# MDFahimAnjum/AliasFree-Diffusion-Models-PyTorch

Measured on AMD Instinct MI355X. Metric: train_step_images_per_sec, higher is better.
Workload: dtype f32; 1 GPU; CIFAR-10 32x32x3 synthetic, UNet variant=3 (Config D), batch 256/GPU, T=1000, AdamW lr 3e-4, random-init weights (seed 42); global_batch=256, parallelism=dp1, hip_graph=True, launch_mode=lanes

## Files before the change

aliasfree-diffusion-models-pytorch_amd/csrc/attn.hip:

```cpp
#include "attn_forms.h"

namespace afd {

constexpr int kTile = 64;
constexpr int kChunk = 8;

using f2 = __attribute__((ext_vector_type(2))) float;
constexpr float kLog2e = 1.4426950408889634f, kLn2 = 0.6931471805599453f;

template <int D> struct RowVec {
  static __device__ __forceinline__ void load(const float* __restrict__ p, f2 (&v)[D / 2]) {
    if constexpr (D % 4 == 0) {
#pragma unroll
      for (int j = 0; j < D / 4; ++j) {
        const float4 t = reinterpret_cast<const float4*>(p)[j];
        v[2 * j] = (f2){t.x, t.y}; v[2 * j + 1] = (f2){t.z, t.w};
      }
    } else {
      const float2 t = *reinterpret_cast<const float2*>(p);
      v[0] = (f2){t.x, t.y};
    }
  }
};
template <int P> __device__ __forceinline__ float dot2(const f2 (&a)[P], const f2 (&b)[P]) {
// ... 145 lines not shown
      const float g = live ? d_o[obase + (long)j * L + qi] : 0.f;
      q[r][j >> 1][j & 1] = live ? qp[(long)j * L + qi] * (scale * kLog2e) : 0.f;
      go[r][j >> 1][j & 1] = g;
      delta[r] += g * (live ? o[obase + (long)j * L + qi] : 0.f);
    }
#pragma unroll
    for (int i = 0; i < P; ++i) dq[r][i] = (f2){0.f, 0.f};
    ls[r] = live ? lse[((long)b * heads + h) * L + qi] * kLog2e : 0.f;
    if (live) delta_out[((long)b * heads + h) * L + qi] = delta[r];
  }
  for (int k0 = 0; k0 < L; k0 += kTile) {
    __syncthreads();
    stage_rows<D, NT>(kp, Ks, k0, L, 1.f);
    stage_rows<D, NT>(vp, Vs, k0, L, 1.f);
    __syncthreads();
    const int nk = min(kTile, L - k0);
#pragma unroll 2
    for (int u = 0; u < nk; ++u) {
      f2 kv[P], vv[P];
      RowVec<D>::load(Ks + u * D, kv);
      RowVec<D>::load(Vs + u * D, vv);
#pragma unroll
      for (int r = 0; r < R; ++r) {
        const float sc = dot2<P>(q[r], kv), dp = dot2<P>(go[r], vv);
        const float ds = __builtin_amdgcn_exp2f(sc - ls[r]) * (dp - delta[r]);
        axpy2<P>(dq[r], ds, kv);
      }
    }
  }
#pragma unroll
  for (int r = 0; r < R; ++r) {
    const int qi = q0 + r * NT;
    if (qi < L) {
      float* dqp = dqkv + ((long)b * 3 * C + h * D) * L + qi;
#pragma unroll
      for (int j = 0; j < D; ++j) dqp[(long)j * L] = dq[r][j >> 1][j & 1] * scale;
    }
  }
}

template <int D, int R, int NT>
__global__ __launch_bounds__(NT) void attn_bwd_dkv_k(const float* __restrict__ qkv, const float* __restrict__ d_o,
                                                      const float* __restrict__ lse, const float* __restrict__ delta,
                                                      float* __restrict__ dqkv, int heads, int L, float scale) {
  constexpr int P = D / 2;
  __shared__ __attribute__((aligned(16))) float Qs[kTile * D];
  __shared__ __attribute__((aligned(16))) float Gs[kTile * D];
  __shared__ float Ls[kTile];
  __shared__ float Ds[kTile];
  const int b = blockIdx.z, h = blockIdx.y;
  const int C = heads * D;
  const int kq0 = blockIdx.x * NT * R + threadIdx.x;
  const float* qp = qkv + ((long)b * 3 * C + h * D) * L;
  const float* kp = qp + (long)C * L;
  const float* vp = kp + (long)C * L;
  const float* gp = d_o + ((long)b * C + h * D) * L;
  const float* lp = lse + ((long)b * heads + h) * L;
  const float* dlp = delta + ((long)b * heads + h) * L;
  f2 k[R][P], v[R][P], dk[R][P], dv[R][P];
#pragma unroll
  for (int r = 0; r < R; ++r) {
    const int ki = kq0 + r * NT;
#pragma unroll
    for (int j = 0; j < D; ++j) {
      k[r][j >> 1][j & 1] = ki < L ? kp[(long)j * L + ki] : 0.f;
      v[r][j >> 1][j & 1] = ki < L ? vp[(long)j * L + ki] : 0.f;
    }
#pragma unroll
    for (int i = 0; i < P; ++i) { dk[r][i] = (f2){0.f, 0.f}; dv[r][i] = (f2){0.f, 0.f}; }
  }
  for (int t0 = 0; t0 < L; t0 += kTile) {
    __syncthreads();
    stage_rows<D, NT>(qp, Qs, t0, L, scale * kLog2e);
    stage_rows<D, NT>(gp, Gs, t0, L, 1.f);
    for (int i = threadIdx.x; i < kTile; i += NT) {
      const bool in = t0 + i < L;
      Ls[i] = in ? lp[t0 + i] * kLog2e : INFINITY;
      Ds[i] = in ? dlp[t0 + i] : 0.f;
    }
    __syncthreads();
    const int nq = min(kTile, L - t0);
#pragma unroll 2
    for (int u = 0; u < nq; ++u) {
      f2 qv[P], gv[P];
      RowVec<D>::load(Qs + u * D, qv);
      RowVec<D>::load(Gs + u * D, gv);
      const float lsu = Ls[u], dlu = Ds[u];
#pragma unroll
      for (int r = 0; r < R; ++r) {
        const float sc = dot2<P>(qv, k[r]), dp = dot2<P>(gv, v[r]);
        const float p = __builtin_amdgcn_exp2f(sc - lsu);
        const float ds = p * (dp - dlu);
        axpy2<P>(dv[r], p, gv);
        axpy2<P>(dk[r], ds, qv);
      }
    }
  }
#pragma unroll
  for (int r = 0; r < R; ++r) {
    const int ki = kq0 + r * NT;
    if (ki < L) {
      float* dkp = dqkv + ((long)b * 3 * C + C + h * D) * L + ki;
      float* dvp = dkp + (long)C * L;
#pragma unroll
      for (int j = 0; j < D; ++j) { dkp[(long)j * L] = dk[r][j >> 1][j & 1] * kLn2; dvp[(long)j * L] = dv[r][j >> 1][j & 1]; }
    }
  }
}

}
using namespace afd;

template <int R> static inline void attn_geometry(int B, int heads, int L, dim3& grid, dim3& block) {
  const int rows = (L + R - 1) / R;
  block = dim3(rows <= 64 ? 64 : (rows <= 128 ? 128 : 256));
  grid = dim3((L + block.x * R - 1) / (block.x * R), heads, B);
}
template <int D, int R> static void launch_fwd(const float* qkv, float* o, float* lse, int B, int heads, int L, float sc, hipStream_t s) {
  dim3 grid, block; attn_geometry<R>(B, heads, L, grid, block);
  if (block.x == 64) hipLaunchKernelGGL((attn_fwd_k<D, R, 64>), grid, block, 0, s, qkv, o, lse, heads, L, sc);
  else if (block.x == 128) hipLaunchKernelGGL((attn_fwd_k<D, R, 128>), grid, block, 0, s, qkv, o, lse, heads, L, sc);
  else hipLaunchKernelGGL((attn_fwd_k<D, R, 256>), grid, block, 0, s, qkv, o, lse, heads, L, sc);
}
template <int D, int R> static void launch_dq(const float* qkv, const float* o, const float* d_o, const float* lse, float* dqkv,
                                              float* delta, int B, int heads, int L, float sc, hipStream_t s) {
  dim3 grid, block; attn_geometry<R>(B, heads, L, grid, block);
  if (block.x == 64) hipLaunchKernelGGL((attn_bwd_dq_k<D, R, 64>), grid, block, 0, s, qkv, o, d_o, lse, dqkv, delta, heads, L, sc);
  else if (block.x == 128) hipLaunchKernelGGL((attn_bwd_dq_k<D, R, 128>), grid, block, 0, s, qkv, o, d_o, lse, dqkv, delta, heads, L, sc);
  else hipLaunchKernelGGL((attn_bwd_dq_k<D, R, 256>), grid, block, 0, s, qkv, o, d_o, lse, dqkv, delta, heads, L, sc);
}
template <int D, int R> static void launch_dkv(const float* qkv, const float* d_o, const float* lse, const float* delta, float* dqkv,
                                               int B, int heads, int L, float sc, hipStream_t s) {
  dim3 grid, block; attn_geometry<R>(B, heads, L, grid, block);
  if (block.x == 64) hipLaunchKernelGGL((attn_bwd_dkv_k<D, R, 64>), grid, block, 0, s, qkv, d_o, lse, delta, dqkv, heads, L, sc);
  else if (block.x == 128) hipLaunchKernelGGL((attn_bwd_dkv_k<D, R, 128>), grid, block, 0, s, qkv, d_o, lse, delta, dqkv, heads, L, sc);
  else hipLaunchKernelGGL((attn_bwd_dkv_k<D, R, 256>), grid, block, 0, s, qkv, d_o, lse, delta, dqkv, heads, L, sc);
}

static int g_attn_mfma_bwd_all = 1;
static int g_attn_rows = 0;

static int g_attn_small = 1;
static inline bool attn_small_use(int B, int heads, int d, int L) {
  return g_attn_small && g_attn_rows == 0 && attn_small_ok(d, L) && (long)B * heads <= (1L << 30);
}

extern "C" {

int afd_debug_attn_rows(int r) {
  if (r == 20 || r == 21) { g_attn_pv = r - 20; return AFD_OK; }
  if (r == 40 || r == 41) { g_attn_pv16 = r - 40; return AFD_OK; }
  if (r == 30 || r == 31) { g_attn_small = r - 30; return AFD_OK; }
  if (r == 10 || r == 11) { g_attn_mfma_bwd_all = r - 10; return AFD_OK; }
  AFD_REQUIRE(r == 0 || r == 1 || r == 2 || r == 4, "afd_debug_attn_rows: r must be 0, 1, 2, 4 (rows per lane of the VALU kernels), 10, 11, 20, 21, 30, 31, 40 or 41");
  g_attn_rows = r;
  return AFD_OK;
}

int afd_attn_fwd(const float* qkv, float* o, float* lse, int B, int heads, int d, int L, afd_stream_t st) {
  AFD_REQUIRE(qkv && o && lse && B > 0 && heads > 0 && L > 0, "afd_attn_fwd: bad argument");
  AFD_REQUIRE(d == 2 || d == 4 || d == 8 || d == 16 || d == 32 || d == 64, "afd_attn_fwd: head dim %d not in {2,4,8,16,32,64}", d);
  AFD_REQUIRE(B <= 65535 && heads <= 65535, "afd_attn_fwd: grid too large");
  hipStream_t s = as_stream(st);
  const float sc = 1.0f / sqrtf((float)d);
  if (g_attn_rows == 0 && attn_mfma8_ok(d, L)) { attn_mfma8_fwd(qkv, o, lse, B, heads, d, L, sc, s); return check_launch("afd_attn_fwd"); }
  if (attn_small_use(B, heads, d, L) && aligned16(qkv)) {
    attn_small_fwd_launch(qkv, o, lse, B, heads, d, L, sc, s);
    return check_launch("afd_attn_fwd");
  }
  switch (d) {
    case 2:  launch_fwd<2, 4>(qkv, o, lse, B, heads, L, sc, s); break;
    case 4:  launch_fwd<4, 4>(qkv, o, lse, B, heads, L, sc, s); break;
    case 8:
      if (g_attn_rows == 1 || (g_attn_rows == 0 && L < 1024)) launch_fwd<8, 1>(qkv, o, lse, B, heads, L, sc, s);
      else if (g_attn_rows == 4) launch_fwd<8, 4>(qkv, o, lse, B, heads, L, sc, s);
      else launch_fwd<8, 2>(qkv, o, lse, B, heads, L, sc, s);
      break;
    case 16: if (L <= 64) launch_fwd<16, 1>(qkv, o, lse, B, heads, L, sc, s); else launch_fwd<16, 2>(qkv, o, lse, B, heads, L, sc, s); break;
    case 32: if (L <= 64) launch_fwd<32, 1>(qkv, o, lse, B, heads, L, sc, s); else launch_fwd<32, 2>(qkv, o, lse, B, heads, L, sc, s); break;
    default: launch_fwd<64, 1>(qkv, o, lse, B, heads, L, sc, s); break;
  }
  return check_launch("afd_attn_fwd");
}

int afd_attn_bwd(const float* qkv, const float* o, const float* d_o, const float* lse, float* dqkv, float* delta_ws,
                 int B, int heads, int d, int L, afd_stream_t st) {
  AFD_REQUIRE(qkv && o && d_o && lse && dqkv && delta_ws && B > 0 && heads > 0 && L > 0, "afd_attn_bwd: bad argument");
  AFD_REQUIRE(d == 2 || d == 4 || d == 8 || d == 16 || d == 32 || d == 64, "afd_attn_bwd: head dim %d not in {2,4,8,16,32,64}", d);
  AFD_REQUIRE(B <= 65535 && heads <= 65535, "afd_attn_bwd: grid too large");
  hipStream_t s = as_stream(st);
  const float sc = 1.0f / sqrtf((float)d);
  if (g_attn_rows == 0 && attn_mfma8_ok(d, L) && (L < 1024 || g_attn_mfma_bwd_all)) {
    if (attn_fused_bwd(qkv, o, d_o, lse, dqkv, delta_ws, B, heads, d, L, sc, s)) return check_launch("afd_attn_bwd");
    attn_mfma8_bwd_dq(qkv, o, d_o, lse, dqkv, delta_ws, B, heads, d, L, sc, s);
    if (d == 8) attn_mfma8_bwd_dkv(qkv, d_o, lse, delta_ws, dqkv, B, heads, L, sc, s);
    else launch_dkv<16, 2>(qkv, d_o, lse, delta_ws, dqkv, B, heads, L, sc, s);
    return check_launch("afd_attn_bwd");
  }
  if (attn_small_use(B, heads, d, L) && aligned16(qkv) && aligned16(d_o)) {
    attn_small_bwd_launch(qkv, d_o, dqkv, B, heads, d, L, sc, s);
    return check_launch("afd_attn_bwd");
  }
  switch (d) {
    case 2:  launch_dq<2, 4>(qkv, o, d_o, lse, dqkv, delta_ws, B, heads, L, sc, s); break;
    case 4:  launch_dq<4, 4>(qkv, o, d_o, lse, dqkv, delta_ws, B, heads, L, sc, s); break;
    case 8:
      if (g_attn_rows == 1 || (g_attn_rows == 0 && L < 1024)) launch_dq<8, 1>(qkv, o, d_o, lse, dqkv, delta_ws, B, heads, L, sc, s);
      else if (g_attn_rows == 4) launch_dq<8, 4>(qkv, o, d_o, lse, dqkv, delta_ws, B, heads, L, sc, s);
      else launch_dq<8, 2>(qkv, o, d_o, lse, dqkv, delta_ws, B, heads, L, sc, s);
      break;
    case 16: if (L <= 64) launch_dq<16, 1>(qkv, o, d_o, lse, dqkv, delta_ws, B, heads, L, sc, s); else launch_dq<16, 2>(qkv, o, d_o, lse, dqkv, delta_ws, B, heads, L, sc, s); break;
    case 32: if (L <= 64) launch_dq<32, 1>(qkv, o, d_o, lse, dqkv, delta_ws, B, heads, L, sc, s); else launch_dq<32, 2>(qkv, o, d_o, lse, dqkv, delta_ws, B, heads, L, sc, s); break;
    default: launch_dq<64, 1>(qkv, o, d_o, lse, dqkv, delta_ws, B, heads, L, sc, s); break;
  }
  switch (d) {
    case 2:  launch_dkv<2, 4>(qkv, d_o, lse, delta_ws, dqkv, B, heads, L, sc, s); break;
    case 4:  launch_dkv<4, 4>(qkv, d_o, lse, delta_ws, dqkv, B, heads, L, sc, s); break;
    case 8:
      if (g_attn_rows == 1 || (g_attn_rows == 0 && L < 1024)) launch_dkv<8, 1>(qkv, d_o, lse, delta_ws, dqkv, B, heads, L, sc, s);
      else if (g_attn_rows == 4) launch_dkv<8, 4>(qkv, d_o, lse, delta_ws, dqkv, B, heads, L, sc, s);
      else launch_dkv<8, 2>(qkv, d_o, lse, delta_ws, dqkv, B, heads, L, sc, s);
      break;
    case 16: if (L <= 64) launch_dkv<16, 1>(qkv, d_o, lse, delta_ws, dqkv, B, heads, L, sc, s); else launch_dkv<16, 2>(qkv, d_o, lse, delta_ws, dqkv, B, heads, L, sc, s); break;
    case 32: launch_dkv<32, 1>(qkv, d_o, lse, delta_ws, dqkv, B, heads, L, sc, s); break;
    default: launch_dkv<64, 1>(qkv, d_o, lse, delta_ws, dqkv, B, heads, L, sc, s); break;
  }
  return check_launch("afd_attn_bwd");
}

}
```

aliasfree-diffusion-models-pytorch_amd/csrc/attn_forms.h:

```cpp
#pragma once
#include "common.h"

namespace afd {

extern int g_attn_pv;
extern int g_attn_pv16;
bool attn_mfma8_ok(int d, int L);
bool attn_fused_bwd(const float* qkv, const float* o, const float* d_o, const float* lse, float* dqkv, float* delta, int B, int heads,
                    int d, int L, float sc, hipStream_t s);
void attn_mfma8_fwd(const float* qkv, float* o, float* lse, int B, int heads, int d, int L, float sc, hipStream_t s);
void attn_mfma8_bwd_dq(const float* qkv, const float* o, const float* d_o, const float* lse, float* dqkv, float* delta,
                       int B, int heads, int d, int L, float sc, hipStream_t s);
void attn_mfma8_bwd_dkv(const float* qkv, const float* d_o, const float* lse, const float* delta, float* dqkv, int B, int heads, int L,
                        float sc, hipStream_t s);

bool attn_small_ok(int d, int L);
void attn_small_fwd_launch(const float* qkv, float* o, float* lse, int B, int heads, int d, int L, float sc, hipStream_t s);
void attn_small_bwd_launch(const float* qkv, const float* d_o, float* dqkv, int B, int heads, int d, int L, float sc, hipStream_t s);

}
```

aliasfree-diffusion-models-pytorch_amd/csrc/attn_mfma.hip:

```cpp
#include "attn_forms.h"
#include "h2_common.h"

namespace afd {

using f32x16 = __attribute__((ext_vector_type(16))) float;
constexpr int kTK = 64;
constexpr float kLog2e = 1.4426950408889634f, kLn2 = 0.6931471805599453f;

__device__ __forceinline__ float xhalf(float v) { return __shfl_xor(v, 32, kWave); }
__device__ __forceinline__ int acc_row(int r, int half) { return (r & 3) + 8 * (r >> 2) + 4 * half; }

using f2 = __attribute__((ext_vector_type(2))) float;
template <int D>
__device__ __forceinline__ void load_row(const float* __restrict__ p, f2 (&v)[D / 2]) {
#pragma unroll
  for (int q = 0; q < D / 4; ++q) {
    const float4 a = reinterpret_cast<const float4*>(p)[q];
    v[2 * q] = (f2){a.x, a.y}; v[2 * q + 1] = (f2){a.z, a.w};
  }
}
template <int D>
__device__ __forceinline__ void axpy(f2 (&acc)[D / 2], float s, const f2 (&v)[D / 2]) {
  const f2 ss = {s, s};
#pragma unroll
  for (int i = 0; i < D / 2; ++i) acc[i] = __builtin_elementwise_fma(ss, v[i], acc[i]);
}

using bf8 = __attribute__((ext_vector_type(8))) __bf16;
using bf2 = __attribute__((ext_vector_type(2))) __bf16;
__device__ __forceinline__ void split3(float x, __bf16& a, __bf16& b, __bf16& c) {
  a = (__bf16)x; const float r = x - (float)a;
  b = (__bf16)r; const float r2 = r - (float)b;
  c = (__bf16)r2;
}
template <int D>
__device__ __forceinline__ void row_frags(const float (&x)[D], int half, bf8 (&f)[3]) {
  bf8 p1, p2, p3;
#pragma unroll
  for (int j = 0; j < 8; ++j) {
    __bf16 a, b, c;
    split3(D == 8 ? x[j] : (half ? x[(8 + j) % D] : x[j]), a, b, c);
    p1[j] = a; p2[j] = b; p3[j] = c;
  }
  if (D == 8) { f[0] = p1; f[1] = half ? p1 : p2; f[2] = half ? p3 : p2; }
  else { f[0] = p1; f[1] = p2; f[2] = p3; }
}
template <int D>
__device__ __forceinline__ void stage_pieces(uint32_t* __restrict__ P, int rr, int jp, float v0, float v1) {
  __bf16 a0, b0, c0, a1, b1, c1;
  split3(v0, a0, b0, c0); split3(v1, a1, b1, c1);
  const int rec = D == 8 ? rr : (jp >> 2) * kTK + rr, w = jp & 3, ps = (D / 8) * kTK;
  P[(0 * ps + rec) * 4 + w] = __builtin_bit_cast(uint32_t, (bf2){a0, a1});
  P[(1 * ps + rec) * 4 + w] = __builtin_bit_cast(uint32_t, (bf2){b0, b1});
  P[(2 * ps + rec) * 4 + w] = __builtin_bit_cast(uint32_t, (bf2){c0, c1});
}
template <int D>
__device__ __forceinline__ void load_frags(const uint32_t* __restrict__ P, int row, int half, bf8 (&a)[3]) {
  const bf8* p = reinterpret_cast<const bf8*>(P);
  if (D == 8) { a[0] = p[(half ? 1 : 0) * kTK + row]; a[1] = p[(half ? 2 : 0) * kTK + row]; a[2] = p[(half ? 0 : 1) * kTK + row]; }
  else {
#pragma unroll
    for (int m = 0; m < 3; ++m) a[m] = p[(m * 2 + half) * kTK + row];
  }
}
template <int D>
__device__ __forceinline__ f32x16 dotx3(const bf8 (&a)[3], const bf8 (&b)[3]) {
  f32x16 c;
#pragma unroll
  for (int r = 0; r < 16; ++r) c[r] = 0.f;
  if (D == 8) {
#pragma unroll
    for (int m = 0; m < 3; ++m) c = __builtin_amdgcn_mfma_f32_32x32x16_bf16(a[m], b[m], c, 0, 0, 0);
  } else {
    constexpr int TA[6] = {0, 1, 0, 2, 1, 0}, TB[6] = {0, 0, 1, 0, 1, 2};
#pragma unroll
    for (int m = 0; m < 6; ++m) c = __builtin_amdgcn_mfma_f32_32x32x16_bf16(a[TA[m]], b[TB[m]], c, 0, 0, 0);
  }
  return c;
}

template <int D>
__device__ __forceinline__ f32x16 dotx3c(const bf8 (&a)[3], const bf8 (&b)[3], f32x16 c) {
  if (D == 8) {
#pragma unroll
    for (int m = 0; m < 3; ++m) c = __builtin_amdgcn_mfma_f32_32x32x16_bf16(a[m], b[m], c, 0, 0, 0);
  } else {
    constexpr int TA[6] = {0, 1, 0, 2, 1, 0}, TB[6] = {0, 0, 1, 0, 1, 2};
#pragma unroll
    for (int m = 0; m < 6; ++m) c = __builtin_amdgcn_mfma_f32_32x32x16_bf16(a[TA[m]], b[TB[m]], c, 0, 0, 0);
  }
  return c;
}

template <int D>
__global__ __launch_bounds__(256, 2) void attn_fwd_mfma(const float* __restrict__ qkv, float* __restrict__ o,
                                                      float* __restrict__ lse, int heads, int L, float scale) {
  __shared__ __attribute__((aligned(16))) uint32_t Kp[3 * (D / 8) * kTK * 4];
  __shared__ __attribute__((aligned(16))) float Vr[kTK * D];
  const int b = blockIdx.z, h = blockIdx.y, C = heads * D;
  const int lane = threadIdx.x & 63, wv = threadIdx.x >> 6, half = lane >> 5, l31 = lane & 31;
  const float* qp = qkv + ((long)b * 3 * C + h * D) * L;
  const float* kp = qp + (long)C * L;
  const float* vp = kp + (long)C * L;
  const int q0 = blockIdx.x * 256 + wv * 64;
  bf8 bq[2][3];
#pragma unroll
  for (int j = 0; j < 2; ++j) {
    float x[D];
#pragma unroll
    for (int d = 0; d < D; ++d) x[d] = qp[(long)d * L + q0 + j * 32 + l31] * (scale * kLog2e);
    row_frags<D>(x, half, bq[j]);
  }
  float m[2] = {-INFINITY, -INFINITY}, l[2] = {0.f, 0.f};
  f2 oa[2][D / 2];
#pragma unroll
  for (int j = 0; j < 2; ++j)
#pragma unroll
    for (int i = 0; i < D / 2; ++i) oa[j][i] = (f2){0.f, 0.f};

  constexpr int NP = D / 8;
  const int jp0 = threadIdx.x >> 6, rr = threadIdx.x & 63;
  float kreg[NP][2], vreg[NP][2];
  auto fetch = [&](int k0) {
#pragma unroll
    for (int e = 0; e < NP; ++e)
#pragma unroll
      for (int h = 0; h < 2; ++h) {
        kreg[e][h] = kp[(long)(2 * (jp0 + 4 * e) + h) * L + k0 + rr];
        vreg[e][h] = vp[(long)(2 * (jp0 + 4 * e) + h) * L + k0 + rr];
      }
  };
  fetch(0);
  for (int k0 = 0; k0 < L; k0 += kTK) {
    __syncthreads();
#pragma unroll
    for (int e = 0; e < NP; ++e) {
      const int jp = jp0 + 4 * e;
      stage_pieces<D>(Kp, rr, jp, kreg[e][0], kreg[e][1]);
      *reinterpret_cast<float2*>(Vr + rr * D + 2 * jp) = make_float2(vreg[e][0], vreg[e][1]);
    }
    __syncthreads();
    if (k0 + kTK < L) fetch(k0 + kTK);
#pragma unroll
    for (int kt = 0; kt < kTK / 32; ++kt) {
      bf8 ak[3];
      load_frags<D>(Kp, kt * 32 + l31, half, ak);
      f32x16 sc[2];
#pragma unroll
      for (int j = 0; j < 2; ++j) {
        sc[j] = dotx3<D>(ak, bq[j]);
        float mx = sc[j][0];
#pragma unroll
        for (int r = 1; r < 16; ++r) mx = fmaxf(mx, sc[j][r]);
        mx = fmaxf(mx, xhalf(mx));
        const float mn = fmaxf(m[j], mx);
        const float alpha = __builtin_amdgcn_exp2f(m[j] - mn);
        l[j] *= alpha;
#pragma unroll
        for (int i = 0; i < D / 2; ++i) oa[j][i] *= alpha;
        m[j] = mn;
      }
#pragma unroll
      for (int r = 0; r < 16; ++r) {
        f2 v[D / 2];
        load_row<D>(Vr + (kt * 32 + acc_row(r, half)) * D, v);
#pragma unroll
        for (int j = 0; j < 2; ++j) {
          const float p = __builtin_amdgcn_exp2f(sc[j][r] - m[j]);
          l[j] += p;
          axpy<D>(oa[j], p, v);
        }
      }
    }
  }
#pragma unroll
  for (int j = 0; j < 2; ++j) {
    const float lt = l[j] + xhalf(l[j]);
    const float inv = 1.0f / lt;
    const int qi = q0 + j * 32 + l31;
#pragma unroll
    for (int d = 0; d < D; ++d) {
      const float mine = oa[j][d >> 1][d & 1];
      const float t = mine + xhalf(mine);
      if (half == 0) o[((long)b * C + h * D + d) * L + qi] = t * inv;
    }
    if (half == 0) lse[((long)b * heads + h) * L + qi] = (m[j] + __builtin_amdgcn_logf(lt)) * kLn2;
  }
}

using h2v = __attribute__((ext_vector_type(2))) _Float16;
using u32x4 = __attribute__((ext_vector_type(4))) uint32_t;
__device__ __forceinline__ float opaque_neg1() {
  float v;
  asm volatile("s_mov_b32 %0, 0xbf800000" : "=s"(v));
  return v;
}
template <bool SUM = false>
__device__ __forceinline__ void pv_split16(const f32x16& sc, float off, float neg1, h8 (&p1)[2], h8 (&p2)[2], float* rowsum = nullptr) {
  const h2v ones = {(_Float16)1.0f, (_Float16)1.0f};
  float s1 = 0.f, s2 = 0.f;
#pragma unroll
  for (int g = 0; g < 2; ++g) {
    u32x4 w1, w2;
#pragma unroll
    for (int q = 0; q < 4; ++q) {
      const float x0 = __builtin_amdgcn_exp2f(sc[8 * g + 2 * q] - off), x1 = __builtin_amdgcn_exp2f(sc[8 * g + 2 * q + 1] - off);
      const h2v a = __builtin_convertvector((f2){x0, x1}, h2v);
      const h2v c = __builtin_convertvector((f2){__builtin_fmaf((float)a[0], neg1, x0), __builtin_fmaf((float)a[1], neg1, x1)}, h2v);
      w1[q] = __builtin_bit_cast(uint32_t, a);
      w2[q] = __builtin_bit_cast(uint32_t, c);
      if (SUM) { s1 = __builtin_amdgcn_fdot2(a, ones, s1, false); s2 = __builtin_amdgcn_fdot2(c, ones, s2, false); }
    }
    p1[g] = __builtin_bit_cast(h8, w1);
    p2[g] = __builtin_bit_cast(h8, w2);
  }
  if (SUM) *rowsum += s1 + s2;
}
__device__ __forceinline__ int a_row16(int d) { return (d & 3) + 8 * ((d >> 2) & 1) + 4 * (d >> 3); }

template <int D>
__global__ __launch_bounds__(256, 2) void attn_fwd_pv(const float* __restrict__ qkv, float* __restrict__ o,
                                                    float* __restrict__ lse, int heads, int L, float scale) {
  static_assert(D == 8 || D == 16, "attn_fwd_pv: head dim 8 or 16");
  constexpr int NP = D / 8, NV = D == 8 ? 8 : 16;
  __shared__ __attribute__((aligned(16))) uint32_t Kp[3 * NP * kTK * 4];
  __shared__ __attribute__((aligned(16))) _Float16 Va[2 * 2 * 2 * 32 * 8];
  __shared__ float wmax[4];
  const int b = blockIdx.z, h = blockIdx.y, C = heads * D;
  const int lane = threadIdx.x & 63, wv = threadIdx.x >> 6, half = lane >> 5, l31 = lane & 31;
  const float* qp = qkv + ((long)b * 3 * C + h * D) * L;
  const float* kp = qp + (long)C * L;
  const float* vp = kp + (long)C * L;
  const int q0 = blockIdx.x * 256 + wv * 64;
  bf8 bq[2][3];
#pragma unroll
  for (int j = 0; j < 2; ++j) {
    float x[D];
#pragma unroll
    for (int d = 0; d < D; ++d) x[d] = qp[(long)d * L + q0 + j * 32 + l31] * (scale * kLog2e);
    row_frags<D>(x, half, bq[j]);
  }
  if (D == 8)
    for (int i = threadIdx.x; i < 2 * 2 * 2 * 16 * 8; i += 256) {
      const int rec = i >> 3, m = 16 + (rec & 15), blk = rec >> 4;
      Va[(blk * 32 + m) * 8 + (i & 7)] = (m == 16 || m == 20) ? (_Float16)1.0f : (_Float16)0.0f;
    }
  float m[2] = {-INFINITY, -INFINITY}, l[2] = {0.f, 0.f};
  f32x16 acc[2];
#pragma unroll
  for (int j = 0; j < 2; ++j)
#pragma unroll
    for (int r = 0; r < 16; ++r) acc[j][r] = 0.f;
  float sv = __uint_as_float(kH2ScaleCapBits);
  const float neg1 = opaque_neg1();

  const int jp0 = threadIdx.x >> 6, rr = threadIdx.x & 63;
  const int rho = rr & 31, vh = (rho >> 2) & 1, vr = (rho & 3) + 4 * (rho >> 3);
  const int vbase = ((((rr >> 5) * 2 + (vr >> 3)) * 2 + vh) * 32) * 8 + (vr & 7);
  float kreg[NP][2], vreg[NP][2];
  auto fetch = [&](int k0) {
#pragma unroll
    for (int e = 0; e < NP; ++e)
#pragma unroll
      for (int hh = 0; hh < 2; ++hh) {
        kreg[e][hh] = kp[(long)(2 * (jp0 + 4 * e) + hh) * L + k0 + rr];
        vreg[e][hh] = vp[(long)(2 * (jp0 + 4 * e) + hh) * L + k0 + rr];
      }
  };
  fetch(0);
  for (int k0 = 0; k0 < L; k0 += kTK) {
    {
      float mv = fmaxf(fabsf(vreg[0][0]), fabsf(vreg[0][1]));
      if (D == 16) mv = fmaxf(mv, fmaxf(fabsf(vreg[NP - 1][0]), fabsf(vreg[NP - 1][1])));
      mv = wave_amax(mv);
      if (lane == 0) wmax[wv] = mv;
    }
    __syncthreads();
    {
      const float sn = fminf(sv, h2_scale_for(fmaxf(fmaxf(wmax[0], wmax[1]), fmaxf(wmax[2], wmax[3]))));
      if (sn != sv) {
        const float f = sn * h2_inv_pow2(sv);
#pragma unroll
        for (int j = 0; j < 2; ++j)
#pragma unroll
          for (int r = 0; r < NV; ++r) acc[j][r] *= f;
        sv = sn;
      }
    }
#pragma unroll
    for (int e = 0; e < NP; ++e) {
      const int jp = jp0 + 4 * e;
      stage_pieces<D>(Kp, rr, jp, kreg[e][0], kreg[e][1]);
#pragma unroll
      for (int hh = 0; hh < 2; ++hh) {
        _Float16 a, c;
        h2_split(vreg[e][hh], sv, a, c);
        const int m1 = D == 8 ? 2 * jp + hh : a_row16(2 * jp + hh);
        Va[vbase + m1 * 8] = a;
        Va[vbase + (m1 + D) * 8] = c;
      }
    }
    __syncthreads();
    if (k0 + kTK < L) fetch(k0 + kTK);
#pragma unroll
    for (int kt = 0; kt < kTK / 32; ++kt) {
      bf8 ak[3];
      load_frags<D>(Kp, kt * 32 + l31, half, ak);
      const h8* va = reinterpret_cast<const h8*>(Va) + ((kt * 2) * 2 + half) * 32 + l31;
      const h8 av0 = va[0], av1 = va[2 * 32];
#pragma unroll
      for (int j = 0; j < 2; ++j) {
        f32x16 sc = dotx3<D>(ak, bq[j]);
        float mx = fmaxf(sc[0], sc[1]);
#pragma unroll
        for (int r = 2; r < 16; r += 2) mx = fmaxf(fmaxf(mx, sc[r]), sc[r + 1]);
        mx = fmaxf(mx, xhalf(mx));
        const float mn = fmaxf(m[j], mx);
        const float alpha = __builtin_amdgcn_exp2f(m[j] - mn);
        m[j] = mn;
#pragma unroll
        for (int r = 0; r < (D == 8 ? 9 : 16); ++r) acc[j][r] *= alpha;
        const float off = mn - 14.0f;
        h8 p1[2], p2[2];
        if (D == 8) pv_split16(sc, off, neg1, p1, p2);
        else { l[j] *= alpha; pv_split16<true>(sc, off, neg1, p1, p2, &l[j]); }
        __builtin_amdgcn_s_setprio(2);
        acc[j] = __builtin_amdgcn_mfma_f32_32x32x16_f16(av0, p1[0], acc[j], 0, 0, 0);
        acc[j] = __builtin_amdgcn_mfma_f32_32x32x16_f16(av1, p1[1], acc[j], 0, 0, 0);
        acc[j] = __builtin_amdgcn_mfma_f32_32x32x16_f16(av0, p2[0], acc[j], 0, 0, 0);
        acc[j] = __builtin_amdgcn_mfma_f32_32x32x16_f16(av1, p2[1], acc[j], 0, 0, 0);
        __builtin_amdgcn_s_setprio(0);
      }
    }
  }
  const float isv = h2_inv_pow2(sv);
#pragma unroll
  for (int j = 0; j < 2; ++j) {
    const float lt = D == 8 ? acc[j][8] : l[j] + xhalf(l[j]);
    const float inv = isv / lt;
    const int qi = q0 + j * 32 + l31;
#pragma unroll
    for (int i = 0; i < D / 2; ++i)
      o[((long)b * C + h * D + (D / 2) * half + i) * L + qi] = (acc[j][i] + acc[j][D / 2 + i]) * inv;
    if (half == 0) lse[((long)b * heads + h) * L + qi] = (m[j] - 14.0f + __builtin_amdgcn_logf(lt)) * kLn2;
  }
}

template <int D, int TJ>
__global__ __launch_bounds__(256, 2) void attn_bwd_dq_mfma(const float* __restrict__ qkv, const float* __restrict__ o,
                                                         const float* __restrict__ d_o, const float* __restrict__ lse,
                                                         float* __restrict__ dqkv, float* __restrict__ delta_out,
                                                         int heads, int L, float scale) {
  __shared__ __attribute__((aligned(16))) uint32_t Kp[3 * (D / 8) * kTK * 4];
  __shared__ __attribute__((aligned(16))) uint32_t Vp[3 * (D / 8) * kTK * 4];
  __shared__ __attribute__((aligned(16))) float Kr[kTK * D];
  const int b = blockIdx.z, h = blockIdx.y, C = heads * D;
  const int lane = threadIdx.x & 63, wv = threadIdx.x >> 6, half = lane >> 5, l31 = lane & 31;
  const float* qp = qkv + ((long)b * 3 * C + h * D) * L;
  const float* kp = qp + (long)C * L;
  const float* vp = kp + (long)C * L;
  const long ob = ((long)b * C + h * D) * L;
  const int q0 = blockIdx.x * (128 * TJ) + wv * (32 * TJ);
  bf8 bq[TJ][3], bg[TJ][3];
  float lsq[TJ], dlt[TJ];
  f2 dq[TJ][D / 2];
#pragma unroll
  for (int j = 0; j < TJ; ++j) {
    const int qi = q0 + j * 32 + l31;
    float dpart = 0.f, xq[D], xg[D];
#pragma unroll
    for (int d = 0; d < D; ++d) {
      xq[d] = qp[(long)d * L + qi] * (scale * kLog2e);
      xg[d] = d_o[ob + (long)d * L + qi];
      dpart = fmaf(xg[d], o[ob + (long)d * L + qi], dpart);
    }
    row_frags<D>(xq, half, bq[j]);
    row_frags<D>(xg, half, bg[j]);
    dlt[j] = dpart;
    lsq[j] = lse[((long)b * heads + h) * L + qi] * kLog2e;
    if (half == 0) delta_out[((long)b * heads + h) * L + qi] = dlt[j];
#pragma unroll
    for (int i = 0; i < D / 2; ++i) dq[j][i] = (f2){0.f, 0.f};
  }
  constexpr int NP = D / 8;
  const int jp0 = threadIdx.x >> 6, rr = threadIdx.x & 63;
  float kreg[NP][2], vreg[NP][2];
  auto fetch = [&](int k0) {
#pragma unroll
    for (int e = 0; e < NP; ++e)
#pragma unroll
      for (int h = 0; h < 2; ++h) {
        kreg[e][h] = kp[(long)(2 * (jp0 + 4 * e) + h) * L + k0 + rr];
        vreg[e][h] = vp[(long)(2 * (jp0 + 4 * e) + h) * L + k0 + rr];
      }
  };
  fetch(0);
  for (int k0 = 0; k0 < L; k0 += kTK) {
    __syncthreads();
#pragma unroll
    for (int e = 0; e < NP; ++e) {
      const int jp = jp0 + 4 * e;
      stage_pieces<D>(Kp, rr, jp, kreg[e][0], kreg[e][1]);
      stage_pieces<D>(Vp, rr, jp, vreg[e][0], vreg[e][1]);
      *reinterpret_cast<float2*>(Kr + rr * D + 2 * jp) = make_float2(kreg[e][0], kreg[e][1]);
    }
    __syncthreads();
    if (k0 + kTK < L) fetch(k0 + kTK);
#pragma unroll
    for (int kt = 0; kt < kTK / 32; ++kt) {
      bf8 ak[3], av[3];
      load_frags<D>(Kp, kt * 32 + l31, half, ak);
      load_frags<D>(Vp, kt * 32 + l31, half, av);
      f32x16 sc[TJ], dp[TJ];
#pragma unroll
      for (int j = 0; j < TJ; ++j) {
        sc[j] = dotx3<D>(ak, bq[j]);
        dp[j] = dotx3<D>(av, bg[j]);
      }
#pragma unroll
      for (int r = 0; r < 16; ++r) {
        f2 kr[D / 2];
        load_row<D>(Kr + (kt * 32 + acc_row(r, half)) * D, kr);
#pragma unroll
        for (int j = 0; j < TJ; ++j) {
          const float ds = __builtin_amdgcn_exp2f(sc[j][r] - lsq[j]) * (dp[j][r] - dlt[j]);
          axpy<D>(dq[j], ds, kr);
        }
      }
    }
  }
#pragma unroll
  for (int j = 0; j < TJ; ++j) {
    const int qi = q0 + j * 32 + l31;
#pragma unroll
    for (int d = 0; d < D; ++d) {
      const float mine = dq[j][d >> 1][d & 1];
      const float t = mine + xhalf(mine);
      if (half == 0) dqkv[((long)b * 3 * C + h * D + d) * L + qi] = t * scale;
    }
  }
}

template <int D, int TJ>
__global__ __launch_bounds__(256, 2) void attn_bwd_dkv_mfma(const float* __restrict__ qkv, const float* __restrict__ d_o,
                                                          const float* __restrict__ lse, const float* __restrict__ delta,
                                                          float* __restrict__ dqkv, int heads, int L, float scale) {
  __shared__ __attribute__((aligned(16))) uint32_t Qp[3 * (D / 8) * kTK * 4];
  __shared__ __attribute__((aligned(16))) uint32_t Gp[3 * (D / 8) * kTK * 4];
  __shared__ __attribute__((aligned(16))) float Qr[kTK * D];
  __shared__ __attribute__((aligned(16))) float Gr[kTK * D];
  __shared__ float Ls[kTK];
  __shared__ float Ds[kTK];
  const int b = blockIdx.z, h = blockIdx.y, C = heads * D;
  const int lane = threadIdx.x & 63, wv = threadIdx.x >> 6, half = lane >> 5, l31 = lane & 31;
  const float* qp = qkv + ((long)b * 3 * C + h * D) * L;
  const float* kp = qp + (long)C * L;
  const float* vp = kp + (long)C * L;
  const float* gp = d_o + ((long)b * C + h * D) * L;
  const float* lp = lse + ((long)b * heads + h) * L;
  const float* dlp = delta + ((long)b * heads + h) * L;
  const int key0 = blockIdx.x * (128 * TJ) + wv * (32 * TJ);
  __shared__ bf8 Bf[4][TJ][2][3][64];
  f2 dk[TJ][D / 2], dv[TJ][D / 2];
#pragma unroll
  for (int j = 0; j < TJ; ++j) {
    float xk[D], xv[D];
#pragma unroll
    for (int d = 0; d < D; ++d) {
      xk[d] = kp[(long)d * L + key0 + j * 32 + l31] * (scale * kLog2e);
      xv[d] = vp[(long)d * L + key0 + j * 32 + l31];
    }
    bf8 t[3];
    row_frags<D>(xk, half, t);
#pragma unroll
    for (int m = 0; m < 3; ++m) Bf[wv][j][0][m][lane] = t[m];
    row_frags<D>(xv, half, t);
#pragma unroll
    for (int m = 0; m < 3; ++m) Bf[wv][j][1][m][lane] = t[m];
#pragma unroll
    for (int i = 0; i < D / 2; ++i) { dk[j][i] = (f2){0.f, 0.f}; dv[j][i] = (f2){0.f, 0.f}; }
  }
  constexpr int NP = D / 8;
  const int jp0 = threadIdx.x >> 6, rr = threadIdx.x & 63;
  float qreg[NP][2], greg[NP][2], lreg = 0.f, dreg = 0.f;
  auto fetch = [&](int t0) {
#pragma unroll
    for (int e = 0; e < NP; ++e)
#pragma unroll
      for (int hh = 0; hh < 2; ++hh) {
        qreg[e][hh] = qp[(long)(2 * (jp0 + 4 * e) + hh) * L + t0 + rr];
        greg[e][hh] = gp[(long)(2 * (jp0 + 4 * e) + hh) * L + t0 + rr];
      }
    if (threadIdx.x < kTK) { lreg = lp[t0 + threadIdx.x] * kLog2e; dreg = dlp[t0 + threadIdx.x]; }
  };
  fetch(0);
  for (int t0 = 0; t0 < L; t0 += kTK) {
    __syncthreads();
// ... 227 lines not shown
      {
        float aq = fmaxf(fabsf(qreg[0][0]), fabsf(qreg[0][1])), ag = fmaxf(fabsf(greg[0][0]), fabsf(greg[0][1]));
        if (D == 16) {
          aq = fmaxf(aq, fmaxf(fabsf(qreg[NP - 1][0]), fabsf(qreg[NP - 1][1])));
          ag = fmaxf(ag, fmaxf(fabsf(greg[NP - 1][0]), fabsf(greg[NP - 1][1])));
        }
        const float mq = wave_amax(aq);
        const float mg = wave_amax(ag);
        const float md = wave_amax(fabsf(dreg));
        if (lane == 0) { wmax[0][wv] = mq; wmax[1][wv] = mg; wmax[2][wv] = md; wmax[3][wv] = v1; }
      }
      __syncthreads();
      const float mq = fmaxf(fmaxf(wmax[0][0], wmax[0][1]), fmaxf(wmax[0][2], wmax[0][3]));
      const float mg = fmaxf(fmaxf(wmax[1][0], wmax[1][1]), fmaxf(wmax[1][2], wmax[1][3]));
      const float md = fmaxf(fmaxf(wmax[2][0], wmax[2][1]), fmaxf(wmax[2][2], wmax[2][3]));
      const float v1g = fmaxf(fmaxf(wmax[3][0], wmax[3][1]), fmaxf(wmax[3][2], wmax[3][3]));
      {
        const float sqn = fminf(sq, h2_scale_for(mq)), sgn = fminf(sg, h2_scale_for(mg));
        const float sdn = fminf(sds, h2_scale_for(fmaf(v1g, mg, md)));
        const float sdc = fminf(sdn, h2_scale_for(mg) * 0x1p64f);
        const float fk = (sqn * h2_inv_pow2(sq)) * (sdc * h2_inv_pow2(sds)), fv = sgn * h2_inv_pow2(sg);
        if (fk != 1.0f || fv != 1.0f) {
#pragma unroll
          for (int j = 0; j < TJ; ++j)
#pragma unroll
            for (int r = 0; r < D; ++r) { accK[j][r] *= fk; accV[j][r] *= fv; }
        }
        sq = sqn; sg = sgn; sds = sdc;
      }
      const float cds = sds * (1.0f / 16384.0f);
#pragma unroll
      for (int e = 0; e < NP; ++e) {
        const int jp = jp0 + 4 * e;
        stage_pieces<D>(Qp, rr, jp, qreg[e][0], qreg[e][1]);
        stage_pieces<D>(Gp, rr, jp, greg[e][0] * cds, greg[e][1] * cds);
#pragma unroll
        for (int hh = 0; hh < 2; ++hh) {
          _Float16 a, c;
          const int m1 = row1(2 * jp + hh);
          h2_split(qreg[e][hh], sq, a, c);
          QA[sbase + m1 * 8] = a; QA[sbase + (m1 + D) * 8] = c;
          h2_split(greg[e][hh], sg, a, c);
          GA[sbase + m1 * 8] = a; GA[sbase + (m1 + D) * 8] = c;
        }
      }
      if (threadIdx.x < kTK) Ls[threadIdx.x] = 14.0f - lreg;
      if (t0 > 0) dq_flush(t0 - kTK);
      if (threadIdx.x < kTK) Ds[threadIdx.x] = -dreg * cds;
      __syncthreads();
      if (t0 + kTK < L) fetch(t0 + kTK);
      const float udq = (scale * h2_inv_pow2(sds)) * h2_inv_pow2(sk);
#pragma unroll
      for (int qt = 0; qt < kTK / 32; ++qt) {
        const h8* qa = reinterpret_cast<const h8*>(QA);
        const h8* ga = reinterpret_cast<const h8*>(GA);
        const h8* ka = reinterpret_cast<const h8*>(KA) + wv * (KREC + ZR);
        f32x16 accQ;
#pragma unroll
        for (int r = 0; r < 16; ++r) accQ[r] = 0.f;
#pragma unroll
        for (int j = 0; j < TJ; ++j) {
          f32x16 sc, dp;
#pragma unroll
          for (int r4 = 0; r4 < 4; ++r4) {
            const int qr = qt * 32 + 8 * r4 + 4 * half;
            const float4 ls = *reinterpret_cast<const float4*>(Ls + qr), dl = *reinterpret_cast<const float4*>(Ds + qr);
            sc[4 * r4] = ls.x; sc[4 * r4 + 1] = ls.y; sc[4 * r4 + 2] = ls.z; sc[4 * r4 + 3] = ls.w;
            dp[4 * r4] = dl.x; dp[4 * r4 + 1] = dl.y; dp[4 * r4 + 2] = dl.z; dp[4 * r4 + 3] = dl.w;
          }
          {
            bf8 aq[3], bkj[3];
            load_frags<D>(Qp, qt * 32 + l31, half, aq);
#pragma unroll
            for (int m = 0; m < 3; ++m) bkj[m] = Bf[wv][j][0][m][lane];
            sc = dotx3c<D>(aq, bkj, sc);
          }
          {
            bf8 ag[3], bvj[3];
            load_frags<D>(Gp, qt * 32 + l31, half, ag);
#pragma unroll
            for (int m = 0; m < 3; ++m) bvj[m] = Bf[wv][j][1][m][lane];
            dp = dotx3c<D>(ag, bvj, dp);
          }
#pragma unroll
          for (int r = 0; r < 16; ++r) {
            const float pv = __builtin_amdgcn_exp2f(sc[r]);
            sc[r] = pv;
            dp[r] *= pv;
          }
          __builtin_amdgcn_sched_barrier(0);
          h8 p1[2], p2[2];
          {
            split16(sc, neg1, p1, p2);
            const h8 ga0 = ga[a_rec(qt, 0, REC)], ga1 = ga[a_rec(qt, 1, REC)];
            __builtin_amdgcn_s_setprio(2);
            accV[j] = __builtin_amdgcn_mfma_f32_32x32x16_f16(ga0, p1[0], accV[j], 0, 0, 0);
            accV[j] = __builtin_amdgcn_mfma_f32_32x32x16_f16(ga1, p1[1], accV[j], 0, 0, 0);
            accV[j] = __builtin_amdgcn_mfma_f32_32x32x16_f16(ga0, p2[0], accV[j], 0, 0, 0);
            accV[j] = __builtin_amdgcn_mfma_f32_32x32x16_f16(ga1, p2[1], accV[j], 0, 0, 0);
          }
          __builtin_amdgcn_s_setprio(0);
          __builtin_amdgcn_sched_barrier(0);
          {
            split16(dp, neg1, p1, p2);
            const h8 qa0 = qa[a_rec(qt, 0, REC)], qa1 = qa[a_rec(qt, 1, REC)];
            __builtin_amdgcn_s_setprio(2);
            accK[j] = __builtin_amdgcn_mfma_f32_32x32x16_f16(qa0, p1[0], accK[j], 0, 0, 0);
            accK[j] = __builtin_amdgcn_mfma_f32_32x32x16_f16(qa1, p1[1], accK[j], 0, 0, 0);
            accK[j] = __builtin_amdgcn_mfma_f32_32x32x16_f16(qa0, p2[0], accK[j], 0, 0, 0);
            accK[j] = __builtin_amdgcn_mfma_f32_32x32x16_f16(qa1, p2[1], accK[j], 0, 0, 0);
          }
          __builtin_amdgcn_sched_barrier(0);
          const h8 ka0 = ka[a_rec(j, 0, KREC)], ka1 = ka[a_rec(j, 1, KREC)];
#pragma unroll
          for (int pc = 0; pc < 2; ++pc) {
            f32x16 t;
#pragma unroll
            for (int r = 0; r < 16; ++r) t[r] = 0.f;
            t = __builtin_amdgcn_mfma_f32_32x32x16_f16(pc ? p2[0] : p1[0], perm[0], t, 0, 0, 0);
            t = __builtin_amdgcn_mfma_f32_32x32x16_f16(pc ? p2[1] : p1[1], perm[1], t, 0, 0, 0);
            h8 e[2];
            pack16(t, e);
            accQ = __builtin_amdgcn_mfma_f32_32x32x16_f16(ka0, e[0], accQ, 0, 0, 0);
            accQ = __builtin_amdgcn_mfma_f32_32x32x16_f16(ka1, e[1], accQ, 0, 0, 0);
          }
          __builtin_amdgcn_s_setprio(0);
          __builtin_amdgcn_sched_barrier(0);
        }
#pragma unroll
        for (int i = 0; i < D / 2; ++i) DQ[wv][(D / 2) * half + i][qt * 32 + l31] = (accQ[i] + accQ[D / 2 + i]) * udq;
      }
    }
    __syncthreads();
    dq_flush(L - kTK);
    {
      const float uk = (scale * h2_inv_pow2(sds)) * h2_inv_pow2(sq), uv = h2_inv_pow2(sg) * (1.0f / 16384.0f);
#pragma unroll
      for (int j = 0; j < TJ; ++j) {
        const int ki = key0 + j * 32 + l31;
#pragma unroll
        for (int i = 0; i < D / 2; ++i) {
          dqkv[((long)b * 3 * C + C + h * D + (D / 2) * half + i) * L + ki] = (accK[j][i] + accK[j][D / 2 + i]) * uk;
          dqkv[((long)b * 3 * C + 2 * C + h * D + (D / 2) * half + i) * L + ki] = (accV[j][i] + accV[j][D / 2 + i]) * uv;
        }
      }
    }
    __syncthreads();
  }
}


bool attn_mfma8_ok(int d, int L) { return (d == 8 || d == 16) && L % 256 == 0; }
int g_attn_pv = 1, g_attn_pv16 = 1;
void attn_mfma8_fwd(const float* qkv, float* o, float* lse, int B, int heads, int d, int L, float sc, hipStream_t s) {
  if (d == 8 && g_attn_pv) hipLaunchKernelGGL(attn_fwd_pv<8>, dim3(L / 256, heads, B), dim3(256), 0, s, qkv, o, lse, heads, L, sc);
  else if (d == 16 && g_attn_pv16) hipLaunchKernelGGL(attn_fwd_pv<16>, dim3(L / 256, heads, B), dim3(256), 0, s, qkv, o, lse, heads, L, sc);
  else if (d == 8) hipLaunchKernelGGL(attn_fwd_mfma<8>, dim3(L / 256, heads, B), dim3(256), 0, s, qkv, o, lse, heads, L, sc);
  else hipLaunchKernelGGL(attn_fwd_mfma<16>, dim3(L / 256, heads, B), dim3(256), 0, s, qkv, o, lse, heads, L, sc);
}
void attn_mfma8_bwd_dq(const float* qkv, const float* o, const float* d_o, const float* lse, float* dqkv, float* delta,
                       int B, int heads, int d, int L, float sc, hipStream_t s) {
  if (d == 8) hipLaunchKernelGGL((attn_bwd_dq_mfma<8, 2>), dim3(L / 256, heads, B), dim3(256), 0, s, qkv, o, d_o, lse, dqkv, delta, heads, L, sc);
  else hipLaunchKernelGGL((attn_bwd_dq_mfma<16, 1>), dim3(L / 128, heads, B), dim3(256), 0, s, qkv, o, d_o, lse, dqkv, delta, heads, L, sc);
}
bool attn_fused_bwd(const float* qkv, const float* o, const float* d_o, const float* lse, float* dqkv, float* delta, int B, int heads,
                    int d, int L, float sc, hipStream_t s) {
  if (!((d == 8 && g_attn_pv) || (d == 16 && g_attn_pv16)) || L % 256) return false;
  const long total = (long)B * heads * L;
  hipLaunchKernelGGL(attn_delta_k, dim3((unsigned)((total + 255) / 256)), dim3(256), 0, s, o, d_o, delta, heads, d, L, total);
  if (d == 8) hipLaunchKernelGGL((attn_bwd_fused<8, 2>), dim3(heads, B), dim3(256), 0, s, qkv, d_o, lse, delta, dqkv, heads, L, sc);
  else hipLaunchKernelGGL((attn_bwd_fused<16, 1>), dim3(heads, B), dim3(256), 0, s, qkv, d_o, lse, delta, dqkv, heads, L, sc);
  return true;
}
void attn_mfma8_bwd_dkv(const float* qkv, const float* d_o, const float* lse, const float* delta, float* dqkv, int B, int heads, int L,
                        float sc, hipStream_t s) {
  hipLaunchKernelGGL((attn_bwd_dkv_mfma<8, 2>), dim3(L / 256, heads, B), dim3(256), 0, s, qkv, d_o, lse, delta, dqkv, heads, L, sc);
}

}
```

Baseline: 40390 images/s.

## Skip online-softmax rescale in attention forward unless row max exceeds threshold

The forward PV attention kernel now folds the running max offset into the MFMA accumulator's initial value, so the scores come out already shifted. The max reduction, accumulator rescale and exp offset are skipped unless some lane's max exceeds a threshold (14 + tau); this is checked with a wave-wide ballot. This removes the per-tile cross-lane shuffle and rescale multiplies on the common path, at the cost of letting exp2 inputs grow up to tau above the reference, which reduces fp16 headroom. The kt loop is also changed from unrolled to unroll 1, which may affect scheduling.

New measurement: 40570 images/s (median of 6 runs). About the same (+0.4%).

```diff
diff --git a/aliasfree-diffusion-models-pytorch_amd/csrc/attn.hip b/aliasfree-diffusion-models-pytorch_amd/csrc/attn.hip
--- a/aliasfree-diffusion-models-pytorch_amd/csrc/attn.hip
+++ b/aliasfree-diffusion-models-pytorch_amd/csrc/attn.hip
@@ -321,7 +321,8 @@
   if (r == 40 || r == 41) { g_attn_pv16 = r - 40; return AFD_OK; }
   if (r == 30 || r == 31) { g_attn_small = r - 30; return AFD_OK; }
   if (r == 10 || r == 11) { g_attn_mfma_bwd_all = r - 10; return AFD_OK; }
-  AFD_REQUIRE(r == 0 || r == 1 || r == 2 || r == 4, "afd_debug_attn_rows: r must be 0, 1, 2, 4 (rows per lane of the VALU kernels), 10, 11, 20, 21, 30, 31, 40 or 41");
+  if (r == 50 || r == 51) { g_attn_fwd_tau = (float)(r - 50); return AFD_OK; }
+  AFD_REQUIRE(r == 0 || r == 1 || r == 2 || r == 4, "afd_debug_attn_rows: r must be 0, 1, 2, 4 (rows per lane of the VALU kernels), 10, 11, 20, 21, 30, 31, 40, 41, 50 or 51");
   g_attn_rows = r;
   return AFD_OK;
 }
diff --git a/aliasfree-diffusion-models-pytorch_amd/csrc/attn_forms.h b/aliasfree-diffusion-models-pytorch_amd/csrc/attn_forms.h
--- a/aliasfree-diffusion-models-pytorch_amd/csrc/attn_forms.h
+++ b/aliasfree-diffusion-models-pytorch_amd/csrc/attn_forms.h
@@ -5,6 +5,7 @@
 
 extern int g_attn_pv;
 extern int g_attn_pv16;
+extern float g_attn_fwd_tau;
 bool attn_mfma8_ok(int d, int L);
 bool attn_fused_bwd(const float* qkv, const float* o, const float* d_o, const float* lse, float* dqkv, float* delta, int B, int heads,
                     int d, int L, float sc, hipStream_t s);
diff --git a/aliasfree-diffusion-models-pytorch_amd/csrc/attn_mfma.hip b/aliasfree-diffusion-models-pytorch_amd/csrc/attn_mfma.hip
--- a/aliasfree-diffusion-models-pytorch_amd/csrc/attn_mfma.hip
+++ b/aliasfree-diffusion-models-pytorch_amd/csrc/attn_mfma.hip
@@ -88,6 +88,21 @@
     constexpr int TA[6] = {0, 1, 0, 2, 1, 0}, TB[6] = {0, 0, 1, 0, 1, 2};
 #pragma unroll
     for (int m = 0; m < 6; ++m) c = __builtin_amdgcn_mfma_f32_32x32x16_bf16(a[TA[m]], b[TB[m]], c, 0, 0, 0);
+  }
+  return c;
+}
+
+template <int D>
+__device__ __forceinline__ f32x16 dotx3k(const bf8 (&a)[3], const bf8 (&b)[3], const f32x16& c0) {
+  f32x16 c;
+  asm("s_nop 1\n\tv_mfma_f32_32x32x16_bf16 %0, %1, %2, %3" : "=&v"(c) : "v"(a[0]), "v"(b[0]), "v"(c0));
+  if (D == 8) {
+#pragma unroll
+    for (int m = 1; m < 3; ++m) c = __builtin_amdgcn_mfma_f32_32x32x16_bf16(a[m], b[m], c, 0, 0, 0);
+  } else {
+    constexpr int TA[6] = {0, 1, 0, 2, 1, 0}, TB[6] = {0, 0, 1, 0, 1, 2};
+#pragma unroll
+    for (int m = 1; m < 6; ++m) c = __builtin_amdgcn_mfma_f32_32x32x16_bf16(a[TA[m]], b[TB[m]], c, 0, 0, 0);
   }
   return c;
 }
@@ -196,7 +211,7 @@
   return v;
 }
 template <bool SUM = false>
-__device__ __forceinline__ void pv_split16(const f32x16& sc, float off, float neg1, h8 (&p1)[2], h8 (&p2)[2], float* rowsum = nullptr) {
+__device__ __forceinline__ void pv_split16(const f32x16& sc, float neg1, h8 (&p1)[2], h8 (&p2)[2], float* rowsum = nullptr) {
   const h2v ones = {(_Float16)1.0f, (_Float16)1.0f};
   float s1 = 0.f, s2 = 0.f;
 #pragma unroll
@@ -204,7 +219,7 @@
     u32x4 w1, w2;
 #pragma unroll
     for (int q = 0; q < 4; ++q) {
-      const float x0 = __builtin_amdgcn_exp2f(sc[8 * g + 2 * q] - off), x1 = __builtin_amdgcn_exp2f(sc[8 * g + 2 * q + 1] - off);
+      const float x0 = __builtin_amdgcn_exp2f(sc[8 * g + 2 * q]), x1 = __builtin_amdgcn_exp2f(sc[8 * g + 2 * q + 1]);
       const h2v a = __builtin_convertvector((f2){x0, x1}, h2v);
       const h2v c = __builtin_convertvector((f2){__builtin_fmaf((float)a[0], neg1, x0), __builtin_fmaf((float)a[1], neg1, x1)}, h2v);
       w1[q] = __builtin_bit_cast(uint32_t, a);
@@ -220,7 +235,7 @@
 
 template <int D>
 __global__ __launch_bounds__(256, 2) void attn_fwd_pv(const float* __restrict__ qkv, float* __restrict__ o,
-                                                    float* __restrict__ lse, int heads, int L, float scale) {
+                                                    float* __restrict__ lse, int heads, int L, float scale, float thr) {
   static_assert(D == 8 || D == 16, "attn_fwd_pv: head dim 8 or 16");
   constexpr int NP = D / 8, NV = D == 8 ? 8 : 16;
   __shared__ __attribute__((aligned(16))) uint32_t Kp[3 * NP * kTK * 4];
@@ -245,12 +260,14 @@
       const int rec = i >> 3, m = 16 + (rec & 15), blk = rec >> 4;
       Va[(blk * 32 + m) * 8 + (i & 7)] = (m == 16 || m == 20) ? (_Float16)1.0f : (_Float16)0.0f;
     }
-  float m[2] = {-INFINITY, -INFINITY}, l[2] = {0.f, 0.f};
-  f32x16 acc[2];
+  float mref[2] = {-INFINITY, -INFINITY}, l[2] = {0.f, 0.f};
+  f32x16 acc[2], cinit[2];
+  float cref[2] = {0.f, 0.f};
+  float thr_now = -INFINITY;
 #pragma unroll
   for (int j = 0; j < 2; ++j)
 #pragma unroll
-    for (int r = 0; r < 16; ++r) acc[j][r] = 0.f;
+    for (int r = 0; r < 16; ++r) { acc[j][r] = 0.f; cinit[j][r] = 0.f; }
   float sv = __uint_as_float(kH2ScaleCapBits);
   const float neg1 = opaque_neg1();
 
@@ -268,6 +285,7 @@
       }
   };
   fetch(0);
+#pragma unroll 1
   for (int k0 = 0; k0 < L; k0 += kTK) {
     {
       float mv = fmaxf(fabsf(vreg[0][0]), fabsf(vreg[0][1]));
@@ -302,7 +320,7 @@
     }
     __syncthreads();
     if (k0 + kTK < L) fetch(k0 + kTK);
-#pragma unroll
+#pragma unroll 1
     for (int kt = 0; kt < kTK / 32; ++kt) {
       bf8 ak[3];
       load_frags<D>(Kp, kt * 32 + l31, half, ak);
@@ -310,20 +328,26 @@
       const h8 av0 = va[0], av1 = va[2 * 32];
 #pragma unroll
       for (int j = 0; j < 2; ++j) {
-        f32x16 sc = dotx3<D>(ak, bq[j]);
+        f32x16 sc = dotx3k<D>(ak, bq[j], cinit[j]);
         float mx = fmaxf(sc[0], sc[1]);
 #pragma unroll
         for (int r = 2; r < 16; r += 2) mx = fmaxf(fmaxf(mx, sc[r]), sc[r + 1]);
-        mx = fmaxf(mx, xhalf(mx));
-        const float mn = fmaxf(m[j], mx);
-        const float alpha = __builtin_amdgcn_exp2f(m[j] - mn);
-        m[j] = mn;
-#pragma unroll
-        for (int r = 0; r < (D == 8 ? 9 : 16); ++r) acc[j][r] *= alpha;
-        const float off = mn - 14.0f;
+        if (__builtin_expect(__builtin_amdgcn_ballot_w64(mx > thr_now) != 0, 0)) {
+          mx = fmaxf(mx, xhalf(mx));
+          const float c = cref[j];
+          const float mn = fmaxf(mref[j], mx - c);
+          const float cn = 14.0f - mn, up = cn - c;
+          const float alpha = mref[j] == -INFINITY ? 0.f : __builtin_amdgcn_exp2f(up);
+          mref[j] = mn; cref[j] = cn;
+#pragma unroll
+          for (int r = 0; r < (D == 8 ? 9 : 16); ++r) acc[j][r] *= alpha;
+          if (D == 16) l[j] *= alpha;
+#pragma unroll
+          for (int r = 0; r < 16; ++r) { sc[r] += up; cinit[j][r] = cn; }
+        }
         h8 p1[2], p2[2];
-        if (D == 8) pv_split16(sc, off, neg1, p1, p2);
-        else { l[j] *= alpha; pv_split16<true>(sc, off, neg1, p1, p2, &l[j]); }
+        if (D == 8) pv_split16(sc, neg1, p1, p2);
+        else pv_split16<true>(sc, neg1, p1, p2, &l[j]);
         __builtin_amdgcn_s_setprio(2);
         acc[j] = __builtin_amdgcn_mfma_f32_32x32x16_f16(av0, p1[0], acc[j], 0, 0, 0);
         acc[j] = __builtin_amdgcn_mfma_f32_32x32x16_f16(av1, p1[1], acc[j], 0, 0, 0);
@@ -331,6 +355,7 @@
         acc[j] = __builtin_amdgcn_mfma_f32_32x32x16_f16(av1, p2[1], acc[j], 0, 0, 0);
         __builtin_amdgcn_s_setprio(0);
       }
+      thr_now = thr;
     }
   }
   const float isv = h2_inv_pow2(sv);
@@ -342,7 +367,7 @@
 #pragma unroll
     for (int i = 0; i < D / 2; ++i)
       o[((long)b * C + h * D + (D / 2) * half + i) * L + qi] = (acc[j][i] + acc[j][D / 2 + i]) * inv;
-    if (half == 0) lse[((long)b * heads + h) * L + qi] = (m[j] - 14.0f + __builtin_amdgcn_logf(lt)) * kLn2;
+    if (half == 0) lse[((long)b * heads + h) * L + qi] = (__builtin_amdgcn_logf(lt) - cref[j]) * kLn2;
   }
 }
 
@@ -876,9 +901,11 @@
 
 bool attn_mfma8_ok(int d, int L) { return (d == 8 || d == 16) && L % 256 == 0; }
 int g_attn_pv = 1, g_attn_pv16 = 1;
+float g_attn_fwd_tau = 1.0f;
 void attn_mfma8_fwd(const float* qkv, float* o, float* lse, int B, int heads, int d, int L, float sc, hipStream_t s) {
-  if (d == 8 && g_attn_pv) hipLaunchKernelGGL(attn_fwd_pv<8>, dim3(L / 256, heads, B), dim3(256), 0, s, qkv, o, lse, heads, L, sc);
-  else if (d == 16 && g_attn_pv16) hipLaunchKernelGGL(attn_fwd_pv<16>, dim3(L / 256, heads, B), dim3(256), 0, s, qkv, o, lse, heads, L, sc);
+  const float thr = 14.0f + g_attn_fwd_tau;
+  if (d == 8 && g_attn_pv) hipLaunchKernelGGL(attn_fwd_pv<8>, dim3(L / 256, heads, B), dim3(256), 0, s, qkv, o, lse, heads, L, sc, thr);
+  else if (d == 16 && g_attn_pv16) hipLaunchKernelGGL(attn_fwd_pv<16>, dim3(L / 256, heads, B), dim3(256), 0, s, qkv, o, lse, heads, L, sc, thr);
   else if (d == 8) hipLaunchKernelGGL(attn_fwd_mfma<8>, dim3(L / 256, heads, B), dim3(256), 0, s, qkv, o, lse, heads, L, sc);
   else hipLaunchKernelGGL(attn_fwd_mfma<16>, dim3(L / 256, heads, B), dim3(256), 0, s, qkv, o, lse, heads, L, sc);
 }
```
